# nghiapq77/face-recognition-cpp-tensorrt

Hardware: AMD Instinct MI355X
Metric: faces/sec end-to-end (detect+embed+match), 640x640 batch=32, 1M gallery (higher is better)
Workload: dtype f16 MFMA recogniser convs (fp32 accumulate) + fp32-accurate detector (fp32 MFMA, fp16 hi/lo-split MFMA for the 64-channel 3x3 convs) + int8-screened coarse scan (fp16 MFMA on exactly widened int8 rows) + exact f32 re-rank match (bit-identical to the exact f32 scan)

## Files before the change

### face-recognition-cpp-tensorrt_amd/csrc/frt_embedder.cpp

```cpp
#include "frt_embedder.hpp"
#include "frt_arc_pack.hpp"
#include "frt_matcher.hpp"

namespace {

using frt::conv_w_f16;
using frt::conv_w_f16_frag;
using frt::conv1x1_w_f16_frag;
std::vector<uint16_t> conv_w_f16(const frt::Blob &b, const std::string &name, int cout, int cin, int ks) {
    return conv_w_f16(b.get(name, (size_t)cout * cin * ks * ks).data, cout, cin, ks);
}
std::vector<float> vec_of(const frt::Blob &b, const std::string &name, size_t n) {
    const float *p = b.get(name, n).data;
    return std::vector<float>(p, p + n);
}


float residual_stream_scale(const frt::Blob &b, const frt::ArcLayout &layout, bool se) {
    if (se || layout.units.size() <= 24) return 1.0f;
    double var = 0.0;
    for (size_t i = 0; i <= layout.units.size(); ++i) {
        const std::string p = i < layout.units.size() ? "body." + std::to_string(i) + ".res_layer.0" : std::string("output_layer.0");
        const frt::Tensor &v = b.get(p + ".running_var", i < layout.units.size() ? layout.units[i].cin : 512);
        for (size_t c = 0; c < v.numel; ++c) var = std::max(var, (double)v.data[c]);
// ... 123 lines not shown
    const size_t F = (size_t)max_batch;
    d_in = arena.alloc<float>(F * 3 * 112 * 112);
    alloc_act_set(act[0]);
    if (se) {
        HIPCHK(hipHostMalloc(reinterpret_cast<void **>(&h_se_error), sizeof(int), hipHostMallocMapped));
        *h_se_error = 0;
        HIPCHK(hipHostGetDevicePointer(reinterpret_cast<void **>(&d_se_error), h_se_error, 0));
    }
    d_out = arena.alloc<float>(F * 512);
    d_crops = arena.alloc<uint8_t>(F * 112 * 112 * 3);
    d_valid = arena.alloc<int>(F);
    d_boxes = arena.alloc<frt_bbox>(F);
    d_lm = arena.alloc<float>((size_t)F * 10);
    zeros = arena.alloc<half_t>(256);
    HIPCHK(hipMemset(zeros, 0, 256 * sizeof(half_t)));
}

void frt_embedder::alloc_act_set(ActSet &a) {
    const size_t F = (size_t)max_batch;
    const size_t big = F * 112 * 112 * 64;
    for (int i = 0; i < 2; ++i) {
        a.Y[i] = arena.alloc<half_t>(big);
        a.Z[i] = arena.alloc<half_t>(big);
    }
    a.T = arena.alloc<half_t>(big);
    a.SC = arena.alloc<half_t>(F * 28 * 28 * 128);
    if (se) {
        a.RES = arena.alloc<half_t>(F * 56 * 56 * 64);
        a.se_pool = arena.alloc<float>(F * 512 * 4 + 2 * F);
        a.se_counter = reinterpret_cast<int *>(a.se_pool + F * 512 * 4);
// ... 672 lines not shown
```

### face-recognition-cpp-tensorrt_amd/csrc/frt_embedder.hpp

```cpp
#pragma once
#include "frt_internal.hpp"

struct ArcUnit {
    int cin, depth, stride, h_in;
    half_t *w1 = nullptr, *w2 = nullptr, *wsc = nullptr;
    half_t *w1f = nullptr, *w2f = nullptr;
    half_t *w2f2 = nullptr;
    half_t *wscf = nullptr;
    float *prelu = nullptr, *s2 = nullptr, *b2 = nullptr, *ssc = nullptr, *bsc = nullptr;
    float *s2f32 = nullptr;
    float *sn = nullptr, *bn = nullptr;
    float *se_w1 = nullptr, *se_w2 = nullptr;
};

struct frt_embedder {
    int device = 0;
    hipStream_t stream = nullptr;
    std::mutex mu;
    hipEvent_t ev_busy[2] = {nullptr, nullptr};
    bool busy[2] = {false, false};
    void wait_idle(hipStream_t s) {
        for (int i = 0; i < 2; ++i)
            if (busy[i]) HIPCHK(hipStreamWaitEvent(s, ev_busy[i], 0));
    }
// ... 55 lines not shown
    struct F32 {
        std::vector<void *> owned;
        std::vector<F32Unit> units;
        float *wfc = nullptr;
        float *A[2] = {nullptr, nullptr}, *T = nullptr, *SCb = nullptr, *RES = nullptr, *gate = nullptr, *fc_out = nullptr;
        int chunk = 0;
        hipEvent_t done = nullptr;
        bool busy = false;
    } f32;
    bool fp32_mode = false;
    std::string blob_path;
    void build_f32();
    void forward_f32(const float *chw_dev, int F, const int *valid_dev, float *out_dev, hipStream_t s);

    void build(const frt::Blob &b);
    void forward(int set, const float *chw_dev, int F, const int *valid_dev, float *out_dev, hipStream_t s);
};

void check_face_images(const frt_face_image *faces, int n, const char *what);
std::vector<frt_face_desc> face_descs(const frt_face_image *faces, int n);
void pack_face_images(const frt_face_image *faces, const frt_face_desc *desc, int first, int count, uint8_t *arena);
```

### face-recognition-cpp-tensorrt_amd/csrc/frt_kernels.h

```cpp
#pragma once
#include <hip/hip_runtime.h>
#include <stdint.h>

#include "../../include/frt.h"
#include "frt_faces.hpp"

typedef _Float16 half_t;
typedef _Float16 half8 __attribute__((ext_vector_type(8)));
typedef _Float16 half4 __attribute__((ext_vector_type(4)));
typedef float floatx16 __attribute__((ext_vector_type(16)));
typedef float floatx4 __attribute__((ext_vector_type(4)));

constexpr int FRT_MAX_DEVICES = 32;
inline bool frt_first_use_on_device(bool (&done)[FRT_MAX_DEVICES]) {
    int d = 0;
    (void)hipGetDevice(&d);
    d &= FRT_MAX_DEVICES - 1;
    if (done[d]) return false;
    done[d] = true;
    return true;
}

void launch_spin(double microseconds, hipStream_t s);
double launch_mfma_probe(int mix, int n_wg, int iters, const void *src, float *out, hipStream_t s);
// ... 195 lines not shown
    int sc_h, sc_w, sc_stride;
    const half_t *scx;
    const half_t *wscf;
    const float *psc0, *psc1;
    int Csc;
    half_t *out0, *out1;
    float *outf;
    int splits;
    const half_t *zeros;
    float *se_pool;
    const float *se_w1, *se_w2;
    int *se_counter;
    int se_flag_off;
    int se_epoch;
    int *se_error;
};
enum ConvFamily { CONV_SMALL, CONV_KS, CONV_C64, CONV_S2, CONV_STRIP };
struct ConvPlan {
    int family = CONV_STRIP;
    int row = 0;
    const char *label = "";
    int R = 0, n_img = 1;
    int M = 0;
    bool uses_scx = false;
    int se_row = -1;
    const char *se_label = nullptr;
    bool se_fused() const { return se_row >= 0; }
    void take_se_tail() { row = se_row; label = se_label; }
};
struct ConvRow {
    const char *label;
    void (*launch)(const ConvMfmaArgs &a, const ConvPlan &p, hipStream_t s);
    int se_row;
};
inline void conv_plan_row(ConvPlan &p, int family, const ConvRow *table, int row) {
    p.family = family;
    p.row = row;
    p.label = table[row].label;
}
inline void conv_plan_se_twin(ConvPlan &p, const ConvRow *table, const ConvMfmaArgs &a) {
    if (table[p.row].se_row < 0 || a.mode != EPI_BN_ADD_BN || !a.se_pool || !a.sc || !a.out1) return;
    p.se_row = table[p.row].se_row;
    p.se_label = table[p.se_row].label;
}
ConvPlan conv_plan(const ConvMfmaArgs &a);
void launch_conv_mfma(const ConvMfmaArgs &a, const ConvPlan &p, hipStream_t s);
bool conv_se_fits_device();
bool plan_small(const ConvMfmaArgs &a, ConvPlan &p);
void launch_small(const ConvMfmaArgs &a, const ConvPlan &p, hipStream_t s);
bool plan_ks(const ConvMfmaArgs &a, ConvPlan &p);
void launch_ks(const ConvMfmaArgs &a, const ConvPlan &p, hipStream_t s);
bool plan_c64(const ConvMfmaArgs &a, ConvPlan &p);
void launch_c64(const ConvMfmaArgs &a, const ConvPlan &p, hipStream_t s);
bool plan_s2(const ConvMfmaArgs &a, ConvPlan &p);
void launch_s2(const ConvMfmaArgs &a, const ConvPlan &p, hipStream_t s);
struct ArcInputArgs {
    const float *x;
    const float *w;
    const float *s0, *b0;
    const float *slope;
// ... 37 lines not shown
```

### face-recognition-cpp-tensorrt_amd/csrc/kernels_arc.hip

```cpp
#include "frt_kernels.h"
#include "frt_se_device.h"

#include <type_traits>

namespace {

__device__ __forceinline__ int swz(int row, int chunk) { return chunk ^ ((row >> 1) & 7); }

template <int WCO, int WPX, int NSTAGE>
__global__ __launch_bounds__(256) void conv_glds_kernel(ConvMfmaArgs p) {
    constexpr int BCO = WCO * 64, BPX = WPX * 64;
    constexpr int CO_CH = BCO * 8 / 256, PX_CH = BPX * 8 / 256;
    constexpr int LPT = CO_CH + PX_CH;
    constexpr int STAGE_HALFS = (BCO + BPX) * 64;
    extern __shared__ __attribute__((aligned(16))) char smem[];
    half_t *ring = reinterpret_cast<half_t *>(smem);

    const int tid = threadIdx.x, lane = tid & 63, wave = tid >> 6;
    const int r = lane & 31, hi = lane >> 5;
    const int wco = wave / WPX, wpx = wave % WPX;

    const int M = p.B * p.Ho * p.Wo;
    const int n_co_tiles = p.Cout / BCO;
    const int nblk = gridDim.x, bq = nblk >> 3, brem = nblk & 7;
// ... 194 lines not shown
    for (int c = threadIdx.x; c < C; c += 256) gate[(long)f * C + c] = se_fc2(shid, w2, C, c);
}

template <int PPS, int PT, int NW, bool SINGLE, bool PAIR, int NT, int BFD, int WR, bool SEP, bool CPT>
__device__ __forceinline__ void conv_patch_body(const ConvMfmaArgs &p, int R, int n_img, int linear) {
    static_assert(!PAIR || SINGLE, "pair mode needs the single-chunk path");
    static_assert(!CPT || (!PAIR && !SINGLE && !SEP && BFD == 1), "compact strips: the main two-buffer variant only (the SE tail pools per image)");
    constexpr int NSLOT = PAIR ? 34 : PT * PPS;
    constexpr int PATCH_B = NSLOT * (PAIR ? 128 : 256) * 16;
    constexpr int PROW = 144;
    extern __shared__ __attribute__((aligned(16))) char smem[];
    const int tid = threadIdx.x, lane = tid & 63, wave = tid >> 6;
    char *patch = smem + (PAIR ? (wave >> 1) * PATCH_B : 0);
    const int r = lane & 31, hi = lane >> 5;
    const int H = p.H, W = p.W, Wp = CPT ? W : W + 2;
    const int NP = CPT ? R * W + 1 : n_img * (R + 2) * Wp;
    const int strips_per_img = (H + R - 1) / R;
    const int n_valid = n_img * R * W;

    const int n_co_tiles = PAIR ? 1 : p.Cout >> 7;
    const int nblk = gridDim.x, bq = nblk >> 3, brem = nblk & 7;
    const int xcd = blockIdx.x & 7, slot = blockIdx.x >> 3;
    const int lid = (xcd < brem ? xcd * (bq + 1) : brem * (bq + 1) + (xcd - brem) * bq) + slot;
    const int co_tile = lid % n_co_tiles;
    const int strip = PAIR ? (lid / n_co_tiles) * 2 + (wave >> 1) : lid / n_co_tiles;
    const int co_base = PAIR ? 0 : co_tile * 128;
    const int cow = PAIR ? (wave & 1) * 32 : wave * 32;
    const int c_mlo = strip * (NT * 32);
    const bool strip_ok = CPT ? c_mlo < p.B * H * W : strip < ((p.B + n_img - 1) / n_img) * strips_per_img;
    const int img0 = CPT ? 0 : (strip / strips_per_img) * n_img;
    const int row0 = CPT ? 0 : (strip % strips_per_img) * R;
    const int c_img_lo = CPT ? c_mlo / (H * W) : 0;
    const int c_rem_lo = CPT ? c_mlo - c_img_lo * (H * W) : 0;
    const int c_top = CPT ? c_img_lo * (H + 1) + c_rem_lo / W - 1 : 0;

    const int n_chunks = p.Cin >> 6;

    int poff[NSLOT];
    {
        const int patch_px = (R + 2) * Wp;
        const float inv_patch = 1.0f / (float)patch_px, inv_wp = 1.0f / (float)Wp;
#pragma unroll
        for (int q = 0; q < NSLOT; ++q) {
            const int g = PAIR ? (q * 2 + (wave & 1)) * 64 + lane : (q * 4 + wave) * 64 + lane;
            const int prow = g / 9, pos = g - prow * 9;
            if constexpr (CPT) {
                const int pp = prow - 1;
                const float inv_w = 1.0f / (float)W, inv_h1 = 1.0f / (float)(H + 1);
                int pr = (int)(((float)pp + 0.5f) * inv_w);
                int pc = pp - pr * W;
                if (pc < 0) { --pr; pc += W; } else if (pc >= W) { ++pr; pc -= W; }
                const int sr = c_top + pr;
                int b = (int)(((float)sr + 0.5f) * inv_h1);
                int iy = sr - b * (H + 1);
                if (iy < 0) { --b; iy += H + 1; } else if (iy > H) { ++b; iy -= H + 1; }
                const bool live = pos < 8 && pp >= 0 && pr < R && strip_ok && sr >= 0 && b < p.B && iy < H;
                poff[q] = live ? ((b * H + iy) * W + pc) * p.Cin + pos * 8 : -1;
                continue;
            }
            int il = (int)(((float)prow + 0.5f) * inv_patch);
            int rem = prow - il * patch_px;
            if (rem < 0) { --il; rem += patch_px; } else if (rem >= patch_px) { ++il; rem -= patch_px; }
            int pr = (int)(((float)rem + 0.5f) * inv_wp);
            int pc = rem - pr * Wp;
            if (pc < 0) { --pr; pc += Wp; } else if (pc >= Wp) { ++pr; pc -= Wp; }
            const int iy = row0 + pr - 1, ix = pc - 1, b = img0 + il;
            const bool live = pos < 8 && prow < NP && strip_ok && b < p.B && iy >= 0 && iy < H && ix >= 0 && ix < W;
            poff[q] = live ? ((b * H + iy) * W + ix) * p.Cin + pos * 8 : -1;
        }
    }
    const half_t *wfrag = p.wf + ((long)((co_base + cow) >> 5) * n_chunks) * (9 * 4 * 512) + lane * 8;
    int pbase[NT];
    unsigned long long mL[CPT ? NT : 1], mR[CPT ? NT : 1];
    const int zoff = hi * 16;
#pragma unroll
    for (int j = 0; j < NT; ++j) {
        const int sl = j * 32 + r;
        int pidx = 0;
        if constexpr (CPT) {
            const int u = c_rem_lo + sl;
            const int per = H * W;
            int il = (int)(((float)u + 0.5f) * (1.0f / (float)per));
            int rem = u - il * per;
            if (rem < 0) { --il; rem += per; } else if (rem >= per) { ++il; rem -= per; }
            int rr = (int)(((float)rem + 0.5f) * (1.0f / (float)W));
            int cc = rem - rr * W;
            if (cc < 0) { --rr; cc += W; } else if (cc >= W) { ++rr; cc -= W; }
            const bool in = c_mlo + sl < p.B * per;
            pidx = in ? ((c_img_lo + il) * (H + 1) + rr - c_top) * W + cc - W : 0;
            mL[j] = __builtin_amdgcn_ballot_w64(cc == 0);
            mR[j] = __builtin_amdgcn_ballot_w64(cc == W - 1);
        } else if (linear) {
            pidx = sl < R * Wp ? sl : 0;
        } else if (sl < n_valid) {
            const int per = R * W;
            int il = (int)(((float)sl + 0.5f) * (1.0f / (float)per));
            int rem = sl - il * per;
            if (rem < 0) { --il; rem += per; } else if (rem >= per) { ++il; rem -= per; }
            int rr = (int)(((float)rem + 0.5f) * (1.0f / (float)W));
            int cc = rem - rr * W;
            if (cc < 0) { --rr; cc += W; } else if (cc >= W) { ++rr; cc -= W; }
            pidx = (il * (R + 2) + rr) * Wp + cc;
        }
        pbase[j] = pidx * PROW + hi * 16;
    }

    half8 areg[WR][4];
    constexpr int LA = WR - 1;
    auto load_w = [&](int c, int tap, auto slot_c) {
        constexpr int S = decltype(slot_c)::value;
        const int woff = c < n_chunks ? (c * 9 + tap) * (4 * 512) : 0;
#pragma unroll
        for (int kk = 0; kk < 4; ++kk) areg[S][kk] = *reinterpret_cast<const half8 *>(wfrag + woff + kk * 512);
    };
    auto issue_patch = [&](int c, auto q0_c, auto nq_c) {
        constexpr int Q0 = decltype(q0_c)::value, NQ = decltype(nq_c)::value;
        const bool real = c < n_chunks;
        char *pl = patch + (SINGLE ? 0 : (c & 1) * PATCH_B) + (PAIR ? (wave & 1) : wave) * 1024;
#pragma unroll
        for (int q = Q0; q < Q0 + NQ; ++q) {
            const half_t *src = (real && poff[q] >= 0) ? p.x + (unsigned)(poff[q] + (c << 6)) : p.zeros;
            __builtin_amdgcn_global_load_lds((const __attribute__((address_space(1))) void *)src,
                                             (__attribute__((address_space(3))) void *)(pl + q * (PAIR ? 2048 : 4096)), 16, 0, 0);
        }
    };

    floatx16 acc[NT];
#pragma unroll
    for (int j = 0; j < NT; ++j)
#pragma unroll
        for (int e = 0; e < 16; ++e) acc[j][e] = 0.f;

    issue_patch(0, std::integral_constant<int, 0>{}, std::integral_constant<int, NSLOT>{});
    load_w(0, 0, std::integral_constant<int, 0>{});
    load_w(0, 1, std::integral_constant<int, 1>{});
    if constexpr (WR == 9) {
        load_w(0, 2, std::integral_constant<int, 2>{});
        load_w(0, 3, std::integral_constant<int, 3>{});
        load_w(0, 4, std::integral_constant<int, 4>{});
        load_w(0, 5, std::integral_constant<int, 5>{});
        load_w(0, 6, std::integral_constant<int, 6>{});
        load_w(0, 7, std::integral_constant<int, 7>{});
    }

    half8 bf[BFD][NT];
    auto frag = [&](int j, auto tap_c, int bufoff, int kko) -> half8 {
        constexpr int T = decltype(tap_c)::value;
        const int dpo = ((T / 3) * Wp + (T % 3)) * PROW + bufoff;
        int a = pbase[j] + dpo;
        if constexpr (CPT && T % 3 == 0) a = __builtin_amdgcn_inverse_ballot_w64(mL[j]) ? zoff + bufoff : a;
        if constexpr (CPT && T % 3 == 2) a = __builtin_amdgcn_inverse_ballot_w64(mR[j]) ? zoff + bufoff : a;
        return *reinterpret_cast<const half8 *>(patch + a + kko * 32);
    };
    asm volatile("s_waitcnt vmcnt(%0)" ::"n"(4 * LA) : "memory");
    __builtin_amdgcn_s_barrier();
#pragma unroll
    for (int k2 = 0; k2 < BFD; ++k2)
#pragma unroll
        for (int j = 0; j < NT; ++j) bf[k2][j] = frag(j, std::integral_constant<int, 0>{}, 0, k2);

    auto step = [&](int c, auto tap_c) {
        constexpr int TAP = decltype(tap_c)::value;
        constexpr int NTAP = (TAP + 1) % 9;
        constexpr int AS = TAP % WR;
        const int pbuf = SINGLE ? 0 : (c & 1) * PATCH_B;
        const int pbufn = TAP == 8 ? (SINGLE ? 0 : ((c + 1) & 1) * PATCH_B) : pbuf;
#pragma unroll
        for (int kk = 0; kk < 4; ++kk) {
            const int cur = BFD == 2 ? (kk & 1) : 0;
// ... 18 lines not shown
                __builtin_amdgcn_sched_barrier(0);
            }
        }
    };
    for (int c = 0; c < n_chunks; ++c) {
        step(c, std::integral_constant<int, 0>{});
        step(c, std::integral_constant<int, 1>{});
        step(c, std::integral_constant<int, 2>{});
        step(c, std::integral_constant<int, 3>{});
        step(c, std::integral_constant<int, 4>{});
        step(c, std::integral_constant<int, 5>{});
        step(c, std::integral_constant<int, 6>{});
        step(c, std::integral_constant<int, 7>{});
        step(c, std::integral_constant<int, 8>{});
    }
    asm volatile("s_waitcnt vmcnt(0)" ::: "memory");
    __syncthreads();

    constexpr int EROW = 36;
    float *ep = reinterpret_cast<float *>(smem) + wave * (32 * EROW);
    const int chunk = lane & 3;
    const int cch = co_base + cow + chunk * 8;
    floatx4 q0[2], q1[2], q2[2], q3[2];
    q0[0] = *reinterpret_cast<const floatx4 *>(p.p0 + cch);
    q0[1] = *reinterpret_cast<const floatx4 *>(p.p0 + cch + 4);
    if (p.mode != EPI_PRELU) {
        q1[0] = *reinterpret_cast<const floatx4 *>(p.p1 + cch);
        q1[1] = *reinterpret_cast<const floatx4 *>(p.p1 + cch + 4);
    }
    if (p.mode == EPI_BN_ADD_BN && p.out1 && !SEP) {
        q2[0] = *reinterpret_cast<const floatx4 *>(p.p2 + cch);
        q2[1] = *reinterpret_cast<const floatx4 *>(p.p2 + cch + 4);
        q3[0] = *reinterpret_cast<const floatx4 *>(p.p3 + cch);
        q3[1] = *reinterpret_cast<const floatx4 *>(p.p3 + cch + 4);
    }
    const long m0 = CPT ? (long)c_mlo : ((long)img0 * H + row0) * W;
    const long Mtot = (long)p.B * H * W;
    const float inv_wp = 1.0f / (float)Wp;
    auto slot_pixel = [&](int sl, long &m) -> bool {
        if constexpr (CPT) {
            m = m0 + sl;
            return m < Mtot;
        }
        if (linear) {
            const int rr = (int)(((float)sl + 0.5f) * inv_wp);
            const int cc = sl - rr * Wp;
            m = m0 + rr * W + cc;
            return strip_ok && rr < R && row0 + rr < H && cc < W && m < Mtot;
        }
        m = m0 + sl;
        return strip_ok && sl < n_valid && m < Mtot;
    };
    if constexpr (SEP) {
        const int per_img = R * W;
        se_tail_epilogue<NT, (NT == 4 ? 2 : 1)>(p, acc, ep, reinterpret_cast<float *>(smem + 4 * 32 * EROW * 4), strip % strips_per_img, strips_per_img,
                                               n_co_tiles, img0, n_img, H * W, co_base, cow, [&](int sl, long &m, int &il) -> bool {
                                                   il = (NT == 4 && !linear && sl >= per_img) ? 1 : 0;
                                                   return slot_pixel(sl, m);
                                               });
        return;
    }
    half8 sc8[NT][2];
    if (p.mode == EPI_BN_ADD_BN) {
#pragma unroll
        for (int j = 0; j < NT; ++j)
#pragma unroll
            for (int it = 0; it < 2; ++it) {
                const int sl = j * 32 + (lane >> 2) + 16 * it;
                long m;
                const bool ok = slot_pixel(sl, m);
                sc8[j][it] = *reinterpret_cast<const half8 *>(p.sc + (ok ? m : 0) * p.Cout + cch);
            }
    }
#pragma unroll
    for (int j = 0; j < NT; ++j) {
#pragma unroll
        for (int g = 0; g < 4; ++g) {
            const floatx4 v = {acc[j][4 * g], acc[j][4 * g + 1], acc[j][4 * g + 2], acc[j][4 * g + 3]};
            *reinterpret_cast<floatx4 *>(ep + r * EROW + 8 * g + 4 * hi) = v;
        }
#pragma unroll
        for (int it = 0; it < 2; ++it) {
            const int px = (lane >> 2) + 16 * it;
            const floatx4 v0 = *reinterpret_cast<const floatx4 *>(ep + px * EROW + chunk * 8);
            const floatx4 v1 = *reinterpret_cast<const floatx4 *>(ep + px * EROW + chunk * 8 + 4);
            const int sl = j * 32 + px;
            long m;
            if (!slot_pixel(sl, m)) continue;
            float v[8] = {v0[0], v0[1], v0[2], v0[3], v1[0], v1[1], v1[2], v1[3]};
            if (p.mode == EPI_PRELU) {
#pragma unroll
                for (int e = 0; e < 8; ++e) v[e] = v[e] > 0.f ? v[e] : v[e] * q0[e >> 2][e & 3];
            } else {
#pragma unroll
                for (int e = 0; e < 8; ++e) v[e] = v[e] * q0[e >> 2][e & 3] + q1[e >> 2][e & 3];
            }
            if (p.mode == EPI_BN_ADD_BN) {
#pragma unroll
                for (int e = 0; e < 8; ++e) v[e] += (float)sc8[j][it][e];
            }
            half8 o;
#pragma unroll
            for (int e = 0; e < 8; ++e) o[e] = (half_t)v[e];
            *reinterpret_cast<half8 *>(p.out0 + m * p.Cout + cch) = o;
            if (p.mode == EPI_BN_ADD_BN && p.out1) {
                half8 z;
#pragma unroll
                for (int e = 0; e < 8; ++e) z[e] = (half_t)(v[e] * q2[e >> 2][e & 3] + q3[e >> 2][e & 3]);
                *reinterpret_cast<half8 *>(p.out1 + m * p.Cout + cch) = z;
            }
        }
    }
}

template <int PPS, int PT, int NW, bool SINGLE, bool PAIR = false, int NT = 7, int BFD = 2, int WR = 3, bool SEP = false>
__global__ __launch_bounds__(256, BFD == 1 ? 2 : 1) void conv_patch_kernel(ConvMfmaArgs p, int R, int n_img, int linear) {
    conv_patch_body<PPS, PT, NW, SINGLE, PAIR, NT, BFD, WR, SEP, false>(p, R, n_img, linear);
}

template <int NT>
__global__ __launch_bounds__(256, 2) void conv_patchc_kernel(ConvMfmaArgs p, int npr) {
    conv_patch_body<10, 1, 5, false, false, NT, 1, 3, false, true>(p, npr, 1, 0);
}

__global__ __launch_bounds__(256) void arc_input_kernel(ArcInputArgs a) {
    __shared__ __attribute__((aligned(16))) float sw[27 * 64 + 5 * 64];
    for (int i = threadIdx.x; i < 27 * 64; i += 256) sw[i] = a.w[i];
// ... 201 lines not shown
            }
            int t = tiles_for(d * (a.W + 2));
            if (!t || t != tiles_for(d * a.W)) t = tiles_for(d * a.W);
            if (!t || !fits(d, 1, t)) continue;
            if (d * a.W * 10 < t * 32 * 7) continue;
            R = d;
            nt = t;
            if (a.B * n_str * co_tiles >= kWant) break;
        }
        if (!R) return false;
    }
    pps = slots_of(R, n_img);
    return true;
}

template <int PPS, int PT, int NW, bool SINGLE, bool PAIR = false, int NT = 7, int BFD = 2, int WR = 3, bool SEP = false>
void launch_patch_t(const ConvMfmaArgs &a, const ConvPlan &p, hipStream_t s) {
    const int R = p.R, n_img = p.n_img;
    const size_t lds = PAIR ? (size_t)2 * 34 * 2048 : (size_t)(SINGLE ? 1 : 2) * PT * PPS * 4096;
    static_assert(PAIR || ((SINGLE ? 1 : 2) * PT * PPS * 4096 <= 160 * 1024 && PT * PPS * 4096 >= 4 * 32 * 36 * 4), "LDS budget / epilogue scratch");
    static bool attr_done[FRT_MAX_DEVICES] = {};
    if (frt_first_use_on_device(attr_done)) {
        (void)hipFuncSetAttribute(reinterpret_cast<const void *>(&conv_patch_kernel<PPS, PT, NW, SINGLE, PAIR, NT, BFD, WR, SEP>), hipFuncAttributeMaxDynamicSharedMemorySize,
                                  (int)lds);
    }
    const int strips = ((a.B + n_img - 1) / n_img) * ((a.H + R - 1) / R);
    dim3 grid(PAIR ? (strips + 1) / 2 : strips * (a.Cout / 128));
    const int linear = (n_img == 1 && R * (a.W + 2) <= NT * 32) ? 1 : 0;
    hipLaunchKernelGGL((conv_patch_kernel<PPS, PT, NW, SINGLE, PAIR, NT, BFD, WR, SEP>), grid, dim3(256), lds, s, a, R, n_img, linear);
}

int compact_patch_rows(const ConvMfmaArgs &a, int nt) {
    const int P = a.H * a.W, S = nt * 32;
    const long M = (long)a.B * P;
    int worst = 0;
    long period = (long)P * S;
    for (long m = 0; m < M && m < period; m += S) {
        const long last = (m + S - 1 < M ? m + S - 1 : M - 1);
        const int sr0 = (int)(m / P) * (a.H + 1) + (int)(m % P) / a.W, sr1 = (int)(last / P) * (a.H + 1) + (int)(last % P) / a.W;
        worst = sr1 - sr0 + 3 > worst ? sr1 - sr0 + 3 : worst;
    }
    return worst;
}

template <int NT>
void launch_patchc_t(const ConvMfmaArgs &a, const ConvPlan &p, hipStream_t s) {
    constexpr size_t lds = (size_t)2 * 10 * 4096;
    static bool attr_done[FRT_MAX_DEVICES] = {};
    if (frt_first_use_on_device(attr_done))
        (void)hipFuncSetAttribute(reinterpret_cast<const void *>(&conv_patchc_kernel<NT>), hipFuncAttributeMaxDynamicSharedMemorySize, (int)lds);
    const long M = (long)a.B * a.H * a.W;
    const int strips = (int)((M + NT * 32 - 1) / (NT * 32));
    hipLaunchKernelGGL((conv_patchc_kernel<NT>), dim3(strips * (a.Cout / 128)), dim3(256), lds, s, a, p.R);
}

enum { CV_G2_22, CV_G2_14, CV_P_PAIR, CV_P_SINGLE, CV_P_255, CV_P_255_SE, CV_P_264, CV_P_255_NT4, CV_P_255_NT4_SE, CV_P_NT2, CV_P_NT1, CV_PC_7, CV_PC_4 };
const ConvRow kStrip[] = {
     {"conv_glds_kernel<2, 2, 2>", launch_glds_t<2, 2, 2>, -1},
     {"conv_glds_kernel<1, 4, 2>", launch_glds_t<1, 4, 2>, -1},
     {"conv_patch_kernel<3, 5, 5, true, true, 7, 2, 3, false>", launch_patch_t<3, 5, 5, true, true>, -1},
     {"conv_patch_kernel<3, 5, 5, true, false, 7, 1, 3, false>", launch_patch_t<3, 5, 5, true, false, 7, 1>, -1},
     {"conv_patch_kernel<10, 1, 5, false, false, 7, 1, 3, false>", launch_patch_t<10, 1, 5, false, false, 7, 1>, CV_P_255_SE},
     {"conv_patch_kernel<10, 1, 5, false, false, 7, 1, 3, true>", launch_patch_t<10, 1, 5, false, false, 7, 1, 3, true>, -1},
     {"conv_patch_kernel<2, 6, 4, false, false, 7, 2, 3, false>", launch_patch_t<2, 6, 4, false>, -1},
     {"conv_patch_kernel<10, 1, 5, false, false, 4, 1, 3, false>", launch_patch_t<10, 1, 5, false, false, 4, 1>, CV_P_255_NT4_SE},
     {"conv_patch_kernel<10, 1, 5, false, false, 4, 1, 3, true>", launch_patch_t<10, 1, 5, false, false, 4, 1, 3, true>, -1},
     {"conv_patch_kernel<5, 1, 5, false, false, 2, 1, 3, false>", launch_patch_t<5, 1, 5, false, false, 2, 1>, -1},
     {"conv_patch_kernel<5, 1, 5, false, false, 1, 1, 3, false>", launch_patch_t<5, 1, 5, false, false, 1, 1>, -1},
     {"conv_patchc_kernel<7>", launch_patchc_t<7>, -1},
     {"conv_patchc_kernel<4>", launch_patchc_t<4>, -1},
};

int strip_variant(const ConvMfmaArgs &a, int &R, int &n_img) {
    int slots, nt;
    bool single;
    if (!patch_geometry(a, R, n_img, slots, single, nt)) return a.Cout % 128 == 0 ? CV_G2_22 : CV_G2_14;
    if (a.Cout == 64) return CV_P_PAIR;
    if (single) return CV_P_SINGLE;
    if (nt == 1) return CV_P_NT1;
    if (nt == 2) return CV_P_NT2;
    const bool epi_ok = a.mode == EPI_PRELU || a.mode == EPI_BN || (a.mode == EPI_BN_ADD_BN && !a.se_pool);
    if (epi_ok && slots <= 10 && ((nt == 7 && n_img == 1 && R == a.H && a.H * a.W < 224) || (nt == 4 && n_img == 2 && 2 * a.H * a.W < 128))) {
        const int npr = compact_patch_rows(a, nt);
        if (npr > 0 && (npr * a.W + 1) * 9 <= 10 * 256) {
            R = npr;
            return nt == 7 ? CV_PC_7 : CV_PC_4;
        }
// ... 9 lines not shown
    p.R = R;
    p.n_img = n_img;
    if (v == CV_P_255 ? (n_img == 1 && a.H / R <= SE_SPLIT) : (v == CV_P_255_NT4 && (n_img == 2 ? R == a.H : a.H / R <= SE_SPLIT))) conv_plan_se_twin(p, kStrip, a);
}

}

ConvPlan conv_plan(const ConvMfmaArgs &a) {
    ConvPlan p;
    if (plan_small(a, p)) return p;
    if (plan_ks(a, p)) return p;
    if (plan_c64(a, p)) return p;
    if (plan_s2(a, p)) return p;
    plan_strip(a, p);
    return p;
}

void launch_conv_mfma(const ConvMfmaArgs &a, const ConvPlan &p, hipStream_t s) {
    switch (p.family) {
        case CONV_SMALL: return launch_small(a, p, s);
        case CONV_KS: return launch_ks(a, p, s);
        case CONV_C64: return launch_c64(a, p, s);
        case CONV_S2: return launch_s2(a, p, s);
        default: return kStrip[p.row].launch(a, p, s);
    }
}

bool conv_se_fits_device() {
    static int ok[FRT_MAX_DEVICES] = {};
    int d = 0;
// ... 33 lines not shown
```

Before: 42790.

## Precompute strip patch/epilogue index tables on host and load them in conv kernels

Replaces the per-thread float-reciprocal index arithmetic in the strip conv kernels (patch gather offsets, B-fragment bases, edge masks, output pixel map) with periodic lookup tables built on the host and cached on device. The tables are warmed at embedder build time for every unit and batch size. The epilogue reads the output slot map from LDS, and its write path is split into full and partial-strip variants. This trades prologue ALU work for extra global loads, and the initial vmcnt wait becomes a full wait.

```diff
diff --git a/face-recognition-cpp-tensorrt_amd/csrc/frt_embedder.cpp b/face-recognition-cpp-tensorrt_amd/csrc/frt_embedder.cpp
--- a/face-recognition-cpp-tensorrt_amd/csrc/frt_embedder.cpp
+++ b/face-recognition-cpp-tensorrt_amd/csrc/frt_embedder.cpp
@@ -161,6 +161,40 @@
     d_lm = arena.alloc<float>((size_t)F * 10);
     zeros = arena.alloc<half_t>(256);
     HIPCHK(hipMemset(zeros, 0, 256 * sizeof(half_t)));
+    warm_strip_tables();
+}
+
+void frt_embedder::warm_strip_tables() {
+    const ActSet &A = act[0];
+    for (const ArcUnit &u : units) {
+        const int h = u.h_in, ho = h / u.stride;
+        for (int F = 1; F <= max_batch; ++F) {
+            ConvMfmaArgs a{};
+            a.x = A.Z[0]; a.w = u.w1; a.wf = u.w1f;
+            a.B = F; a.H = h; a.W = h; a.Cin = u.cin; a.Ho = h; a.Wo = h; a.Cout = u.depth; a.ks = 3; a.stride = 1; a.pad = 1;
+            a.mode = EPI_PRELU;
+            a.out0 = A.T;
+            a.splits = 1;
+            conv_strip_tables_warm(a, conv_plan(a));
+            ConvMfmaArgs c{};
+            c.x = A.T; c.w = u.w2; c.wf = u.w2f; c.wf2 = u.w2f2;
+            c.B = F; c.H = h; c.W = h; c.Cin = u.depth; c.Ho = ho; c.Wo = ho; c.Cout = u.depth; c.ks = 3; c.stride = u.stride; c.pad = 1;
+            c.splits = 1;
+            c.mode = EPI_BN_ADD_BN;
+            c.sc = A.Y[0];
+            c.sc_h = h; c.sc_w = h; c.sc_stride = u.stride;
+            if (&u == &units[0] || u.wsc) c.sc_h = ho, c.sc_w = ho, c.sc_stride = 1;
+            c.out0 = A.Y[1]; c.out1 = A.Z[1];
+            if (se) c.se_pool = A.se_pool, c.se_w1 = u.se_w1, c.se_w2 = u.se_w2, c.se_counter = A.se_counter;
+            conv_strip_tables_warm(c, conv_plan(c));
+            if (se) {
+                ConvMfmaArgs f = c;
+                f.mode = EPI_BN;
+                f.out0 = A.RES; f.out1 = nullptr; f.sc = nullptr;
+                conv_strip_tables_warm(f, conv_plan(f));
+            }
+        }
+    }
 }
 
 void frt_embedder::alloc_act_set(ActSet &a) {
diff --git a/face-recognition-cpp-tensorrt_amd/csrc/frt_embedder.hpp b/face-recognition-cpp-tensorrt_amd/csrc/frt_embedder.hpp
--- a/face-recognition-cpp-tensorrt_amd/csrc/frt_embedder.hpp
+++ b/face-recognition-cpp-tensorrt_amd/csrc/frt_embedder.hpp
@@ -93,6 +93,7 @@
     void forward_f32(const float *chw_dev, int F, const int *valid_dev, float *out_dev, hipStream_t s);
 
     void build(const frt::Blob &b);
+    void warm_strip_tables();
     void forward(int set, const float *chw_dev, int F, const int *valid_dev, float *out_dev, hipStream_t s);
 };
 
diff --git a/face-recognition-cpp-tensorrt_amd/csrc/frt_kernels.h b/face-recognition-cpp-tensorrt_amd/csrc/frt_kernels.h
--- a/face-recognition-cpp-tensorrt_amd/csrc/frt_kernels.h
+++ b/face-recognition-cpp-tensorrt_amd/csrc/frt_kernels.h
@@ -1,6 +1,8 @@
 #pragma once
 #include <hip/hip_runtime.h>
 #include <stdint.h>
+
+#include <vector>
 
 #include "../../include/frt.h"
 #include "frt_faces.hpp"
@@ -233,7 +235,27 @@
     int se_flag_off;
     int se_epoch;
     int *se_error;
-};
+    const int *strip_tab;
+    int strip_period, strip_ppx;
+};
+struct StripGeometry {
+    int H, W;
+    int compact;
+    int linear;
+    int nt;
+    int R;
+    int n_img;
+    int nslot;
+    int threads;
+};
+struct StripTables {
+    int period = 0;
+    int ppx = 0;
+    int stride = 0;
+    std::vector<int> data;
+};
+constexpr int strip_table_stride(const StripGeometry &g) { return g.nslot * g.threads + g.nt * 64 + (g.compact ? g.nt * 4 : g.nt * 32); }
+StripTables strip_tables(const StripGeometry &g);
 enum ConvFamily { CONV_SMALL, CONV_KS, CONV_C64, CONV_S2, CONV_STRIP };
 struct ConvPlan {
     int family = CONV_STRIP;
@@ -263,6 +285,8 @@
     p.se_label = table[p.se_row].label;
 }
 ConvPlan conv_plan(const ConvMfmaArgs &a);
+bool conv_strip_geometry(const ConvMfmaArgs &a, const ConvPlan &p, StripGeometry &g);
+void conv_strip_tables_warm(const ConvMfmaArgs &a, const ConvPlan &p);
 void launch_conv_mfma(const ConvMfmaArgs &a, const ConvPlan &p, hipStream_t s);
 bool conv_se_fits_device();
 bool plan_small(const ConvMfmaArgs &a, ConvPlan &p);
diff --git a/face-recognition-cpp-tensorrt_amd/csrc/kernels_arc.hip b/face-recognition-cpp-tensorrt_amd/csrc/kernels_arc.hip
--- a/face-recognition-cpp-tensorrt_amd/csrc/kernels_arc.hip
+++ b/face-recognition-cpp-tensorrt_amd/csrc/kernels_arc.hip
@@ -1,7 +1,14 @@
 #include "frt_kernels.h"
 #include "frt_se_device.h"
 
+#include <array>
+#include <map>
+#include <mutex>
+#include <stdexcept>
+#include <string>
 #include <type_traits>
+#include <utility>
+#include <vector>
 
 namespace {
 
@@ -232,9 +239,6 @@
     char *patch = smem + (PAIR ? (wave >> 1) * PATCH_B : 0);
     const int r = lane & 31, hi = lane >> 5;
     const int H = p.H, W = p.W, Wp = CPT ? W : W + 2;
-    const int NP = CPT ? R * W + 1 : n_img * (R + 2) * Wp;
-    const int strips_per_img = (H + R - 1) / R;
-    const int n_valid = n_img * R * W;
 
     const int n_co_tiles = PAIR ? 1 : p.Cout >> 7;
     const int nblk = gridDim.x, bq = nblk >> 3, brem = nblk & 7;
@@ -244,84 +248,24 @@
     const int strip = PAIR ? (lid / n_co_tiles) * 2 + (wave >> 1) : lid / n_co_tiles;
     const int co_base = PAIR ? 0 : co_tile * 128;
     const int cow = PAIR ? (wave & 1) * 32 : wave * 32;
+    const int per_idx = strip / p.strip_period, sp = strip - per_idx * p.strip_period;
+    const int pix_off = per_idx * p.strip_ppx;
+    const int Mpix = p.B * H * W;
+    const int img0 = CPT ? 0 : per_idx * n_img;
     const int c_mlo = strip * (NT * 32);
-    const bool strip_ok = CPT ? c_mlo < p.B * H * W : strip < ((p.B + n_img - 1) / n_img) * strips_per_img;
-    const int img0 = CPT ? 0 : (strip / strips_per_img) * n_img;
-    const int row0 = CPT ? 0 : (strip % strips_per_img) * R;
-    const int c_img_lo = CPT ? c_mlo / (H * W) : 0;
-    const int c_rem_lo = CPT ? c_mlo - c_img_lo * (H * W) : 0;
-    const int c_top = CPT ? c_img_lo * (H + 1) + c_rem_lo / W - 1 : 0;
+    const bool strip_ok = CPT ? c_mlo < Mpix : pix_off < Mpix;
+    constexpr int TTHR = PAIR ? 128 : 256;
+    constexpr int T_PBASE = NSLOT * TTHR, T_TAIL = T_PBASE + NT * 64, T_STRIDE = T_TAIL + (CPT ? NT * 4 : NT * 32);
+    const int *__restrict__ tab = p.strip_tab + sp * T_STRIDE;
+    const int tt = PAIR ? (wave & 1) * 64 + lane : tid;
 
     const int n_chunks = p.Cin >> 6;
 
+    const half_t *wfrag = p.wf + ((long)((co_base + cow) >> 5) * n_chunks) * (9 * 4 * 512) + lane * 8;
     int poff[NSLOT];
-    {
-        const int patch_px = (R + 2) * Wp;
-        const float inv_patch = 1.0f / (float)patch_px, inv_wp = 1.0f / (float)Wp;
-#pragma unroll
-        for (int q = 0; q < NSLOT; ++q) {
-            const int g = PAIR ? (q * 2 + (wave & 1)) * 64 + lane : (q * 4 + wave) * 64 + lane;
-            const int prow = g / 9, pos = g - prow * 9;
-            if constexpr (CPT) {
-                const int pp = prow - 1;
-                const float inv_w = 1.0f / (float)W, inv_h1 = 1.0f / (float)(H + 1);
-                int pr = (int)(((float)pp + 0.5f) * inv_w);
-                int pc = pp - pr * W;
-                if (pc < 0) { --pr; pc += W; } else if (pc >= W) { ++pr; pc -= W; }
-                const int sr = c_top + pr;
-                int b = (int)(((float)sr + 0.5f) * inv_h1);
-                int iy = sr - b * (H + 1);
-                if (iy < 0) { --b; iy += H + 1; } else if (iy > H) { ++b; iy -= H + 1; }
-                const bool live = pos < 8 && pp >= 0 && pr < R && strip_ok && sr >= 0 && b < p.B && iy < H;
-                poff[q] = live ? ((b * H + iy) * W + pc) * p.Cin + pos * 8 : -1;
-                continue;
-            }
-            int il = (int)(((float)prow + 0.5f) * inv_patch);
-            int rem = prow - il * patch_px;
-            if (rem < 0) { --il; rem += patch_px; } else if (rem >= patch_px) { ++il; rem -= patch_px; }
-            int pr = (int)(((float)rem + 0.5f) * inv_wp);
-            int pc = rem - pr * Wp;
-            if (pc < 0) { --pr; pc += Wp; } else if (pc >= Wp) { ++pr; pc -= Wp; }
-            const int iy = row0 + pr - 1, ix = pc - 1, b = img0 + il;
-            const bool live = pos < 8 && prow < NP && strip_ok && b < p.B && iy >= 0 && iy < H && ix >= 0 && ix < W;
-            poff[q] = live ? ((b * H + iy) * W + ix) * p.Cin + pos * 8 : -1;
-        }
-    }
-    const half_t *wfrag = p.wf + ((long)((co_base + cow) >> 5) * n_chunks) * (9 * 4 * 512) + lane * 8;
     int pbase[NT];
     unsigned long long mL[CPT ? NT : 1], mR[CPT ? NT : 1];
     const int zoff = hi * 16;
-#pragma unroll
-    for (int j = 0; j < NT; ++j) {
-        const int sl = j * 32 + r;
-        int pidx = 0;
-        if constexpr (CPT) {
-            const int u = c_rem_lo + sl;
-            const int per = H * W;
-            int il = (int)(((float)u + 0.5f) * (1.0f / (float)per));
-            int rem = u - il * per;
-            if (rem < 0) { --il; rem += per; } else if (rem >= per) { ++il; rem -= per; }
-            int rr = (int)(((float)rem + 0.5f) * (1.0f / (float)W));
-            int cc = rem - rr * W;
-            if (cc < 0) { --rr; cc += W; } else if (cc >= W) { ++rr; cc -= W; }
-            const bool in = c_mlo + sl < p.B * per;
-            pidx = in ? ((c_img_lo + il) * (H + 1) + rr - c_top) * W + cc - W : 0;
-            mL[j] = __builtin_amdgcn_ballot_w64(cc == 0);
-            mR[j] = __builtin_amdgcn_ballot_w64(cc == W - 1);
-        } else if (linear) {
-            pidx = sl < R * Wp ? sl : 0;
-        } else if (sl < n_valid) {
-            const int per = R * W;
-            int il = (int)(((float)sl + 0.5f) * (1.0f / (float)per));
-            int rem = sl - il * per;
-            if (rem < 0) { --il; rem += per; } else if (rem >= per) { ++il; rem -= per; }
-            int rr = (int)(((float)rem + 0.5f) * (1.0f / (float)W));
-            int cc = rem - rr * W;
-            if (cc < 0) { --rr; cc += W; } else if (cc >= W) { ++rr; cc -= W; }
-            pidx = (il * (R + 2) + rr) * Wp + cc;
-        }
-        pbase[j] = pidx * PROW + hi * 16;
-    }
 
     half8 areg[WR][4];
     constexpr int LA = WR - 1;
@@ -349,7 +293,6 @@
 #pragma unroll
         for (int e = 0; e < 16; ++e) acc[j][e] = 0.f;
 
-    issue_patch(0, std::integral_constant<int, 0>{}, std::integral_constant<int, NSLOT>{});
     load_w(0, 0, std::integral_constant<int, 0>{});
     load_w(0, 1, std::integral_constant<int, 1>{});
     if constexpr (WR == 9) {
@@ -360,6 +303,33 @@
         load_w(0, 6, std::integral_constant<int, 6>{});
         load_w(0, 7, std::integral_constant<int, 7>{});
     }
+    {
+#pragma unroll
+        for (int q = 0; q < NSLOT; ++q) poff[q] = tab[q * TTHR + tt];
+#pragma unroll
+        for (int j = 0; j < NT; ++j) pbase[j] = tab[T_PBASE + j * 64 + lane];
+        if constexpr (CPT) {
+            const unsigned long long *__restrict__ tm = reinterpret_cast<const unsigned long long *>(tab + T_TAIL);
+#pragma unroll
+            for (int j = 0; j < NT; ++j) {
+                mL[j] = tm[2 * j];
+                mR[j] = tm[2 * j + 1];
+            }
+        }
+        const int t9 = tt % 9;
+#pragma unroll
+        for (int q = 0; q < NSLOT; ++q) {
+            int pos = t9 + (q * TTHR) % 9;
+            pos = pos >= 9 ? pos - 9 : pos;
+            const int px = poff[q] + pix_off;
+            poff[q] = (poff[q] >= 0 && strip_ok && px < Mpix) ? px * p.Cin + pos * 8 : -1;
+        }
+        if constexpr (CPT) {
+#pragma unroll
+            for (int j = 0; j < NT; ++j) pbase[j] = c_mlo + j * 32 + r < Mpix ? pbase[j] : zoff;
+        }
+    }
+    issue_patch(0, std::integral_constant<int, 0>{}, std::integral_constant<int, NSLOT>{});
 
     half8 bf[BFD][NT];
     auto frag = [&](int j, auto tap_c, int bufoff, int kko) -> half8 {
@@ -370,7 +340,7 @@
         if constexpr (CPT && T % 3 == 2) a = __builtin_amdgcn_inverse_ballot_w64(mR[j]) ? zoff + bufoff : a;
         return *reinterpret_cast<const half8 *>(patch + a + kko * 32);
     };
-    asm volatile("s_waitcnt vmcnt(%0)" ::"n"(4 * LA) : "memory");
+    asm volatile("s_waitcnt vmcnt(0)" ::: "memory");
     __builtin_amdgcn_s_barrier();
 #pragma unroll
     for (int k2 = 0; k2 < BFD; ++k2)
@@ -419,10 +389,25 @@
         step(c, std::integral_constant<int, 7>{});
         step(c, std::integral_constant<int, 8>{});
     }
+    constexpr int EROW = 36;
+    constexpr int ESLOTS = (NT * 32 + TTHR - 1) / TTHR;
+    int *eL = reinterpret_cast<int *>(smem + 4 * 32 * EROW * 4 + (576 + 2 * 128) * 4) + (PAIR ? (wave >> 1) * (NT * 32) : 0);
+    static_assert(4 * 32 * EROW * 4 + (576 + 2 * 128) * 4 + 2 * 7 * 32 * 4 <= 2 * 5 * 4096, "slot map behind the epilogue scratch of the smallest patch buffer pair");
+    int ev[ESLOTS];
+    (void)ev;
+    if constexpr (!CPT) {
+#pragma unroll
+        for (int i = 0; i < ESLOTS; ++i) ev[i] = tt + i * TTHR < NT * 32 ? tab[T_TAIL + tt + i * TTHR] : -1;
+    }
     asm volatile("s_waitcnt vmcnt(0)" ::: "memory");
     __syncthreads();
-
-    constexpr int EROW = 36;
+    if constexpr (!CPT) {
+#pragma unroll
+        for (int i = 0; i < ESLOTS; ++i)
+            if (tt + i * TTHR < NT * 32) eL[tt + i * TTHR] = ev[i];
+        __syncthreads();
+    }
+
     float *ep = reinterpret_cast<float *>(smem) + wave * (32 * EROW);
     const int chunk = lane & 3;
     const int cch = co_base + cow + chunk * 8;
@@ -439,83 +424,94 @@
         q3[0] = *reinterpret_cast<const floatx4 *>(p.p3 + cch);
         q3[1] = *reinterpret_cast<const floatx4 *>(p.p3 + cch + 4);
     }
-    const long m0 = CPT ? (long)c_mlo : ((long)img0 * H + row0) * W;
-    const long Mtot = (long)p.B * H * W;
-    const float inv_wp = 1.0f / (float)Wp;
-    auto slot_pixel = [&](int sl, long &m) -> bool {
+    const int mbase = CPT ? c_mlo : pix_off;
+    const bool full = CPT ? c_mlo + NT * 32 <= Mpix : pix_off + p.strip_ppx <= Mpix;
+    auto slot_rel = [&](int sl, auto full_c, int &rel) -> bool {
+        constexpr bool FULL = decltype(full_c)::value;
         if constexpr (CPT) {
-            m = m0 + sl;
-            return m < Mtot;
-        }
-        if (linear) {
-            const int rr = (int)(((float)sl + 0.5f) * inv_wp);
-            const int cc = sl - rr * Wp;
-            m = m0 + rr * W + cc;
-            return strip_ok && rr < R && row0 + rr < H && cc < W && m < Mtot;
-        }
-        m = m0 + sl;
-        return strip_ok && sl < n_valid && m < Mtot;
+            rel = sl;
+            return FULL || mbase + rel < Mpix;
+        }
+        rel = eL[sl];
+        return rel >= 0 && (FULL || mbase + rel < Mpix);
     };
     if constexpr (SEP) {
         const int per_img = R * W;
-        se_tail_epilogue<NT, (NT == 4 ? 2 : 1)>(p, acc, ep, reinterpret_cast<float *>(smem + 4 * 32 * EROW * 4), strip % strips_per_img, strips_per_img,
+        se_tail_epilogue<NT, (NT == 4 ? 2 : 1)>(p, acc, ep, reinterpret_cast<float *>(smem + 4 * 32 * EROW * 4), sp, p.strip_period,
                                                n_co_tiles, img0, n_img, H * W, co_base, cow, [&](int sl, long &m, int &il) -> bool {
                                                    il = (NT == 4 && !linear && sl >= per_img) ? 1 : 0;
-                                                   return slot_pixel(sl, m);
+                                                   int rel;
+                                                   const bool ok = slot_rel(sl, std::false_type{}, rel);
+                                                   m = (long)mbase + rel;
+                                                   return ok;
                                                });
         return;
     }
-    half8 sc8[NT][2];
-    if (p.mode == EPI_BN_ADD_BN) {
-#pragma unroll
-        for (int j = 0; j < NT; ++j)
+    const size_t wbase = (size_t)mbase * p.Cout;
+    half_t *const o0 = p.out0 + wbase;
+    half_t *const o1 = p.out1 ? p.out1 + wbase : nullptr;
+    const half_t *const scw = p.mode == EPI_BN_ADD_BN ? p.sc + wbase : nullptr;
+    const unsigned lane_off = (unsigned)((lane >> 2) * p.Cout + cch);
+    auto write_out = [&](auto full_c) {
+        constexpr bool FULL = decltype(full_c)::value;
+        auto offset_of = [&](int j, int it, int rel) -> unsigned {
+            if constexpr (CPT) return (unsigned)((j * 32 + 16 * it) * p.Cout) + lane_off;
+            return (unsigned)(rel * p.Cout + cch);
+        };
+        half8 sc8[NT][2];
+        if (p.mode == EPI_BN_ADD_BN) {
+#pragma unroll
+            for (int j = 0; j < NT; ++j)
+#pragma unroll
+                for (int it = 0; it < 2; ++it) {
+                    int rel;
+                    const bool ok = slot_rel(j * 32 + (lane >> 2) + 16 * it, full_c, rel);
+                    if constexpr (CPT && FULL) sc8[j][it] = *reinterpret_cast<const half8 *>(scw + offset_of(j, it, rel));
+                    else sc8[j][it] = *reinterpret_cast<const half8 *>(ok ? scw + offset_of(j, it, rel) : p.sc + cch);
+                }
+        }
+#pragma unroll
+        for (int j = 0; j < NT; ++j) {
+#pragma unroll
+            for (int g = 0; g < 4; ++g) {
+                const floatx4 v = {acc[j][4 * g], acc[j][4 * g + 1], acc[j][4 * g + 2], acc[j][4 * g + 3]};
+                *reinterpret_cast<floatx4 *>(ep + r * EROW + 8 * g + 4 * hi) = v;
+            }
 #pragma unroll
             for (int it = 0; it < 2; ++it) {
-                const int sl = j * 32 + (lane >> 2) + 16 * it;
-                long m;
-                const bool ok = slot_pixel(sl, m);
-                sc8[j][it] = *reinterpret_cast<const half8 *>(p.sc + (ok ? m : 0) * p.Cout + cch);
-            }
-    }
-#pragma unroll
-    for (int j = 0; j < NT; ++j) {
-#pragma unroll
-        for (int g = 0; g < 4; ++g) {
-            const floatx4 v = {acc[j][4 * g], acc[j][4 * g + 1], acc[j][4 * g + 2], acc[j][4 * g + 3]};
-            *reinterpret_cast<floatx4 *>(ep + r * EROW + 8 * g + 4 * hi) = v;
-        }
-#pragma unroll
-        for (int it = 0; it < 2; ++it) {
-            const int px = (lane >> 2) + 16 * it;
-            const floatx4 v0 = *reinterpret_cast<const floatx4 *>(ep + px * EROW + chunk * 8);
-            const floatx4 v1 = *reinterpret_cast<const floatx4 *>(ep + px * EROW + chunk * 8 + 4);
-            const int sl = j * 32 + px;
-            long m;
-            if (!slot_pixel(sl, m)) continue;
-            float v[8] = {v0[0], v0[1], v0[2], v0[3], v1[0], v1[1], v1[2], v1[3]};
-            if (p.mode == EPI_PRELU) {
-#pragma unroll
-                for (int e = 0; e < 8; ++e) v[e] = v[e] > 0.f ? v[e] : v[e] * q0[e >> 2][e & 3];
-            } else {
-#pragma unroll
-                for (int e = 0; e < 8; ++e) v[e] = v[e] * q0[e >> 2][e & 3] + q1[e >> 2][e & 3];
-            }
-            if (p.mode == EPI_BN_ADD_BN) {
-#pragma unroll
-                for (int e = 0; e < 8; ++e) v[e] += (float)sc8[j][it][e];
-            }
-            half8 o;
-#pragma unroll
-            for (int e = 0; e < 8; ++e) o[e] = (half_t)v[e];
-            *reinterpret_cast<half8 *>(p.out0 + m * p.Cout + cch) = o;
-            if (p.mode == EPI_BN_ADD_BN && p.out1) {
-                half8 z;
-#pragma unroll
-                for (int e = 0; e < 8; ++e) z[e] = (half_t)(v[e] * q2[e >> 2][e & 3] + q3[e >> 2][e & 3]);
-                *reinterpret_cast<half8 *>(p.out1 + m * p.Cout + cch) = z;
-            }
-        }
-    }
+                const int px = (lane >> 2) + 16 * it;
+                const floatx4 v0 = *reinterpret_cast<const floatx4 *>(ep + px * EROW + chunk * 8);
+                const floatx4 v1 = *reinterpret_cast<const floatx4 *>(ep + px * EROW + chunk * 8 + 4);
+                int rel;
+                if (!slot_rel(j * 32 + px, full_c, rel)) continue;
+                const unsigned off = offset_of(j, it, rel);
+                float v[8] = {v0[0], v0[1], v0[2], v0[3], v1[0], v1[1], v1[2], v1[3]};
+                if (p.mode == EPI_PRELU) {
+#pragma unroll
+                    for (int e = 0; e < 8; ++e) v[e] = v[e] > 0.f ? v[e] : v[e] * q0[e >> 2][e & 3];
+                } else {
+#pragma unroll
+                    for (int e = 0; e < 8; ++e) v[e] = v[e] * q0[e >> 2][e & 3] + q1[e >> 2][e & 3];
+                }
+                if (p.mode == EPI_BN_ADD_BN) {
+#pragma unroll
+                    for (int e = 0; e < 8; ++e) v[e] += (float)sc8[j][it][e];
+                }
+                half8 o;
+#pragma unroll
+                for (int e = 0; e < 8; ++e) o[e] = (half_t)v[e];
+                *reinterpret_cast<half8 *>(o0 + off) = o;
+                if (p.mode == EPI_BN_ADD_BN && p.out1) {
+                    half8 z;
+#pragma unroll
+                    for (int e = 0; e < 8; ++e) z[e] = (half_t)(v[e] * q2[e >> 2][e & 3] + q3[e >> 2][e & 3]);
+                    *reinterpret_cast<half8 *>(o1 + off) = z;
+                }
+            }
+        }
+    };
+    if (full) write_out(std::true_type{});
+    else write_out(std::false_type{});
 }
 
 template <int PPS, int PT, int NW, bool SINGLE, bool PAIR = false, int NT = 7, int BFD = 2, int WR = 3, bool SEP = false>
@@ -747,6 +743,54 @@
     return true;
 }
 
+struct StripTabDev {
+    const int *dev;
+    int period, ppx;
+};
+StripTabDev strip_tab_device(const StripGeometry &g, hipStream_t s = nullptr) {
+    static std::mutex mu;
+    static std::map<std::array<int, 10>, StripTabDev> cache;
+    thread_local std::vector<std::pair<std::array<int, 10>, StripTabDev>> mine;
+    int d = 0;
+    (void)hipGetDevice(&d);
+    const std::array<int, 10> key = {d, g.H, g.W, g.compact, g.linear, g.nt, g.R, g.n_img, g.nslot, g.threads};
+    for (const auto &e : mine)
+        if (e.first == key) return e.second;
+    std::lock_guard<std::mutex> lock(mu);
+    auto it = cache.find(key);
+    if (it == cache.end()) {
+        hipStreamCaptureStatus cap = hipStreamCaptureStatusNone;
+        if (s && hipStreamIsCapturing(s, &cap) == hipSuccess && cap != hipStreamCaptureStatusNone)
+            throw std::runtime_error("strip tables: first use of a strip geometry inside a stream capture (frt_embedder::build() warms every geometry it plans)");
+        const StripTables t = strip_tables(g);
+        int *dev = nullptr;
+        if (hipMalloc(reinterpret_cast<void **>(&dev), t.data.size() * sizeof(int)) != hipSuccess ||
+            hipMemcpy(dev, t.data.data(), t.data.size() * sizeof(int), hipMemcpyHostToDevice) != hipSuccess)
+            throw std::runtime_error("strip tables: device allocation or copy failed");
+        it = cache.emplace(key, StripTabDev{dev, t.period, t.ppx}).first;
+    }
+    mine.emplace_back(key, it->second);
+    return it->second;
+}
+ConvMfmaArgs with_strip_tables(const ConvMfmaArgs &a, const StripGeometry &g, hipStream_t s) {
+    if ((long)a.B * a.H * a.W * a.Cin >= (1L << 31)) throw std::runtime_error("strip kernel: the input tensor exceeds 32-bit element offsets");
+    const StripTabDev t = strip_tab_device(g, s);
+    ConvMfmaArgs b = a;
+    b.strip_tab = t.dev;
+    b.strip_period = t.period;
+    b.strip_ppx = t.ppx;
+    return b;
+}
+template <int PPS, int PT, bool PAIR, int NT>
+StripGeometry patch_strip_geometry(const ConvMfmaArgs &a, const ConvPlan &p) {
+    const int linear = (p.n_img == 1 && p.R * (a.W + 2) <= NT * 32) ? 1 : 0;
+    return StripGeometry{a.H, a.W, 0, linear, NT, p.R, p.n_img, PAIR ? 34 : PT * PPS, PAIR ? 128 : 256};
+}
+template <int NT>
+StripGeometry patchc_strip_geometry(const ConvMfmaArgs &a, const ConvPlan &p) {
+    return StripGeometry{a.H, a.W, 1, 0, NT, p.R, 1, 10, 256};
+}
+
 template <int PPS, int PT, int NW, bool SINGLE, bool PAIR = false, int NT = 7, int BFD = 2, int WR = 3, bool SEP = false>
 void launch_patch_t(const ConvMfmaArgs &a, const ConvPlan &p, hipStream_t s) {
     const int R = p.R, n_img = p.n_img;
@@ -759,8 +803,8 @@
     }
     const int strips = ((a.B + n_img - 1) / n_img) * ((a.H + R - 1) / R);
     dim3 grid(PAIR ? (strips + 1) / 2 : strips * (a.Cout / 128));
-    const int linear = (n_img == 1 && R * (a.W + 2) <= NT * 32) ? 1 : 0;
-    hipLaunchKernelGGL((conv_patch_kernel<PPS, PT, NW, SINGLE, PAIR, NT, BFD, WR, SEP>), grid, dim3(256), lds, s, a, R, n_img, linear);
+    const StripGeometry g = patch_strip_geometry<PPS, PT, PAIR, NT>(a, p);
+    hipLaunchKernelGGL((conv_patch_kernel<PPS, PT, NW, SINGLE, PAIR, NT, BFD, WR, SEP>), grid, dim3(256), lds, s, with_strip_tables(a, g, s), R, n_img, g.linear);
 }
 
 int compact_patch_rows(const ConvMfmaArgs &a, int nt) {
@@ -784,7 +828,7 @@
         (void)hipFuncSetAttribute(reinterpret_cast<const void *>(&conv_patchc_kernel<NT>), hipFuncAttributeMaxDynamicSharedMemorySize, (int)lds);
     const long M = (long)a.B * a.H * a.W;
     const int strips = (int)((M + NT * 32 - 1) / (NT * 32));
-    hipLaunchKernelGGL((conv_patchc_kernel<NT>), dim3(strips * (a.Cout / 128)), dim3(256), lds, s, a, p.R);
+    hipLaunchKernelGGL((conv_patchc_kernel<NT>), dim3(strips * (a.Cout / 128)), dim3(256), lds, s, with_strip_tables(a, patchc_strip_geometry<NT>(a, p), s), p.R);
 }
 
 enum { CV_G2_22, CV_G2_14, CV_P_PAIR, CV_P_SINGLE, CV_P_255, CV_P_255_SE, CV_P_264, CV_P_255_NT4, CV_P_255_NT4_SE, CV_P_NT2, CV_P_NT1, CV_PC_7, CV_PC_4 };
@@ -804,6 +848,24 @@
      {"conv_patchc_kernel<4>", launch_patchc_t<4>, -1},
 };
 
+typedef StripGeometry (*StripGeometryFn)(const ConvMfmaArgs &, const ConvPlan &);
+const StripGeometryFn kStripGeometry[] = {
+     nullptr,
+     nullptr,
+     patch_strip_geometry<3, 5, true, 7>,
+     patch_strip_geometry<3, 5, false, 7>,
+     patch_strip_geometry<10, 1, false, 7>,
+     patch_strip_geometry<10, 1, false, 7>,
+     patch_strip_geometry<2, 6, false, 7>,
+     patch_strip_geometry<10, 1, false, 4>,
+     patch_strip_geometry<10, 1, false, 4>,
+     patch_strip_geometry<5, 1, false, 2>,
+     patch_strip_geometry<5, 1, false, 1>,
+     patchc_strip_geometry<7>,
+     patchc_strip_geometry<4>,
+};
+static_assert(sizeof(kStripGeometry) / sizeof(kStripGeometry[0]) == sizeof(kStrip) / sizeof(kStrip[0]), "one geometry per row");
+
 int strip_variant(const ConvMfmaArgs &a, int &R, int &n_img) {
     int slots, nt;
     bool single;
@@ -843,6 +905,117 @@
     if (plan_s2(a, p)) return p;
     plan_strip(a, p);
     return p;
+}
+
+bool conv_strip_geometry(const ConvMfmaArgs &a, const ConvPlan &p, StripGeometry &g) {
+    if (p.family != CONV_STRIP || !kStripGeometry[p.row]) return false;
+    g = kStripGeometry[p.row](a, p);
+    return true;
+}
+
+void conv_strip_tables_warm(const ConvMfmaArgs &a, const ConvPlan &p) {
+    StripGeometry g;
+    if (conv_strip_geometry(a, p, g)) (void)strip_tab_device(g);
+    if (p.se_fused()) {
+        ConvPlan q = p;
+        q.take_se_tail();
+        if (conv_strip_geometry(a, q, g)) (void)strip_tab_device(g);
+    }
+}
+
+StripTables strip_tables(const StripGeometry &g) {
+    const int H = g.H, W = g.W, NT = g.nt, R = g.R, T = g.threads, P = H * W, S = NT * 32;
+    auto bad = [](const char *what) { throw std::runtime_error(std::string("strip tables: ") + what); };
+    if (H < 1 || W < 1 || NT < 1 || R < 1 || g.n_img < 1 || g.nslot < 1 || (T != 128 && T != 256)) bad("geometry");
+    StripTables t;
+    t.stride = strip_table_stride(g);
+    const int o_pbase = g.nslot * T, o_tail = o_pbase + NT * 64;
+    const int patch_bytes = g.nslot * T * 16, PROW = 144;
+    const int Wp = g.compact ? W : W + 2;
+    if (g.compact) {
+        int a = P, b = S;
+        while (b) { const int c = a % b; a = b; b = c; }
+        t.period = P / a;
+        t.ppx = t.period * S;
+    } else {
+        t.period = (H + R - 1) / R;
+        t.ppx = g.n_img * P;
+    }
+    t.data.assign((size_t)t.period * t.stride, -1);
+    for (int sp = 0; sp < t.period; ++sp) {
+        int *blk = t.data.data() + (size_t)sp * t.stride;
+        const int mlo = sp * S, img_lo = mlo / P, rem_lo = mlo % P;
+        const int top = img_lo * (H + 1) + rem_lo / W - 1;
+        const int row0 = sp * R;
+        const int patch_px = (R + 2) * Wp;
+        for (int q = 0; q < g.nslot; ++q)
+            for (int tt = 0; tt < T; ++tt) {
+                const int piece = q * T + tt, prow = piece / 9, pos = piece % 9;
+                int e = -1;
+                if (g.compact) {
+                    const int pp = prow - 1;
+                    if (pos < 8 && pp >= 0 && pp / W < R && top + pp / W >= 0) {
+                        const int sr = top + pp / W, b = sr / (H + 1), iy = sr % (H + 1);
+                        if (iy < H) e = (b * H + iy) * W + pp % W;
+                    }
+                } else if (pos < 8 && prow < g.n_img * patch_px) {
+                    const int il = prow / patch_px, rem = prow % patch_px;
+                    const int iy = row0 + rem / Wp - 1, ix = rem % Wp - 1;
+                    if (iy >= 0 && iy < H && ix >= 0 && ix < W) e = (il * H + iy) * W + ix;
+                }
+                if (e < -1 || e >= t.ppx + (g.compact ? R * W : 0)) bad("input pixel outside the period");
+                blk[q * T + tt] = e;
+            }
+        for (int j = 0; j < NT; ++j) {
+            unsigned long long mL = 0, mR = 0;
+            for (int lane = 0; lane < 64; ++lane) {
+                const int r = lane & 31, hi = lane >> 5, sl = j * 32 + r;
+                int pidx = 0;
+                bool first = false, last = false;
+                if (g.compact) {
+                    const int u = rem_lo + sl, il = u / P, rem = u % P, rr = rem / W, cc = rem % W;
+                    pidx = ((img_lo + il) * (H + 1) + rr - top) * W + cc - W;
+                    first = cc == 0;
+                    last = cc == W - 1;
+                    if ((mlo + sl) % P % W != cc) bad("column of a compact slot");
+                } else if (g.linear) {
+                    pidx = sl < R * Wp ? sl : 0;
+                } else if (sl < g.n_img * R * W) {
+                    const int per = R * W, il = sl / per, rem = sl % per;
+                    pidx = (il * (R + 2) + rem / W) * Wp + rem % W;
+                }
+                const int pb = pidx * PROW + hi * 16;
+                for (int tap = 0; tap < 9; ++tap) {
+                    if ((tap % 3 == 0 && first) || (tap % 3 == 2 && last)) continue;
+                    const int at = pb + ((tap / 3) * Wp + tap % 3) * PROW;
+                    if (at < 0 || at + 3 * 32 + 16 > patch_bytes) bad("B fragment outside the patch buffer");
+                }
+                blk[o_pbase + j * 64 + lane] = pb;
+                if (first) mL |= 1ull << lane;
+                if (last) mR |= 1ull << lane;
+            }
+            if (g.compact) {
+                if ((mL >> 32) != (mL & 0xffffffffull) || (mR >> 32) != (mR & 0xffffffffull)) bad("mask halves differ");
+                blk[o_tail + 4 * j + 0] = (int)(mL & 0xffffffffull);
+                blk[o_tail + 4 * j + 1] = (int)(mL >> 32);
+                blk[o_tail + 4 * j + 2] = (int)(mR & 0xffffffffull);
+                blk[o_tail + 4 * j + 3] = (int)(mR >> 32);
+            }
+        }
+        if (!g.compact)
+            for (int sl = 0; sl < S; ++sl) {
+                int e = -1;
+                if (g.linear) {
+                    const int rr = sl / Wp, cc = sl % Wp;
+                    if (rr < R && row0 + rr < H && cc < W) e = (row0 + rr) * W + cc;
+                } else if (sl < g.n_img * R * W) {
+                    e = row0 * W + sl;
+                }
+                if (e < -1 || e >= t.ppx) bad("output pixel outside the period");
+                blk[o_tail + sl] = e;
+            }
+    }
+    return t;
 }
 
 void launch_conv_mfma(const ConvMfmaArgs &a, const ConvPlan &p, hipStream_t s) {
```

Measured after the change: 43650, median of 6. 2.0% higher.
